# Leonhard111/M3L

Measured on NVIDIA B200. Metric: VTMAE train samples/sec (fwd+bwd+AdamW), higher is better.
Workload: dtype bf16

## Files before the change

### include/m3l_b200.h

```cpp
#ifndef M3L_B200_H_
#define M3L_B200_H_

#include <stddef.h>
#include <stdint.h>

#ifdef __cplusplus
extern "C" {
#endif

const char* m3l_last_error(void);

typedef struct m3l_gemm_args {
  const void* a;
  const void* b;
  int32_t lda, ldb;
  int32_t a_mn_major;
  int32_t b_mn_major;
  int32_t m, n, k;
  int32_t splits;
  int32_t bn;
  void* out;
  int32_t ldo;
  int32_t out_mode;
  const float* bias;
// ... 24 lines not shown
int m3l_gemm_bf16(const m3l_gemm_args* args, void* stream);


typedef struct m3l_ln_mlp_args {
  const void* x;
  int32_t rows, dim, hidden;
  const float* gamma;
  const float* beta;
  float eps;
  const void* w1;
  const float* b1;
  const void* w2;
  const float* b2;
  void* out;
  int32_t out_has_x;
  float* stats;
  void* xn_out;
  void* h_out;
  void* gp_out;
} m3l_ln_mlp_args;

int m3l_ln_mlp_fwd(const m3l_ln_mlp_args* args, void* stream);

#define M3L_MAX_SEGMENTS 8
typedef struct m3l_mask_segments {
  int32_t count;
  int32_t offset[M3L_MAX_SEGMENTS];
  int32_t length[M3L_MAX_SEGMENTS];
  int32_t n_masked[M3L_MAX_SEGMENTS];
} m3l_mask_segments;

int m3l_mask_indices(const float* noise, int batch, int n_total, const m3l_mask_segments* segs,
                     int64_t* masked, int64_t* unmasked, int32_t* slot_of_token,
                     int32_t* unmasked_i32, int32_t* masked_row_of_token, int n_masked_first,
                     void* stream);

typedef struct m3l_patch_source {
  const void* src[4];
  int32_t channels, height, width, patch_h, patch_w;
  int32_t token_base;
  int32_t layout;
  int32_t dtype;
  int64_t stride_b;
  int32_t chan_group;
  int32_t stride_f, stride_ch, stride_y, stride_x;
  float norm_lo, norm_span;
// ... 117 lines not shown
```

### m3l_b200/_lib.py

```python
from __future__ import annotations

import ctypes as C
import os
from pathlib import Path

_LIB_PATH = Path(os.environ.get("M3L_B200_LIB") or (Path(__file__).resolve().parent / "lib" / "libm3l_b200.so"))
_lib = None


class M3LError(RuntimeError):
    pass


class GemmArgs(C.Structure):
    _fields_ = [
        ("a", C.c_void_p), ("b", C.c_void_p),
        ("lda", C.c_int32), ("ldb", C.c_int32),
        ("a_mn_major", C.c_int32), ("b_mn_major", C.c_int32),
        ("m", C.c_int32), ("n", C.c_int32), ("k", C.c_int32),
        ("splits", C.c_int32), ("bn", C.c_int32),
        ("out", C.c_void_p), ("ldo", C.c_int32), ("out_mode", C.c_int32),
        ("bias", C.c_void_p), ("residual", C.c_void_p), ("ldr", C.c_int32),
        ("act", C.c_int32), ("aux_out", C.c_void_p), ("aux_in", C.c_void_p),
        ("ld_aux", C.c_int32), ("alpha", C.c_float), ("colsum_out", C.c_void_p),
        ("out2", C.c_void_p), ("dot_side", C.c_void_p), ("ld_dot", C.c_int32), ("dot_out", C.c_void_p),
        ("ln_x", C.c_void_p), ("ln_stats", C.c_void_p), ("ln_gamma", C.c_void_p), ("ln_skip", C.c_void_p),
        ("ln_dgamma", C.c_void_p), ("ln_dbeta", C.c_void_p), ("ln_dxcol", C.c_void_p),
        ("drop_key", C.c_void_p), ("drop_site", C.c_int32), ("drop_p", C.c_float),
    ]


class LnMlpArgs(C.Structure):
    _fields_ = [
        ("x", C.c_void_p), ("rows", C.c_int32), ("dim", C.c_int32), ("hidden", C.c_int32),
        ("gamma", C.c_void_p), ("beta", C.c_void_p), ("eps", C.c_float),
        ("w1", C.c_void_p), ("b1", C.c_void_p), ("w2", C.c_void_p), ("b2", C.c_void_p),
        ("out", C.c_void_p), ("out_has_x", C.c_int32), ("stats", C.c_void_p), ("xn_out", C.c_void_p),
        ("h_out", C.c_void_p), ("gp_out", C.c_void_p),
    ]


def lib_path() -> Path:
    return _LIB_PATH


def load() -> C.CDLL:
    global _lib
    if _lib is not None:
        return _lib
    if not _LIB_PATH.exists():
        if os.environ.get("M3L_B200_AUTOBUILD", "0") == "1":
            from . import build as _build

            _build.build(verbose=False)
        else:
            raise M3LError(
                f"{_LIB_PATH} not found: the CUDA extension is not built. Run "
                "`python -m m3l_b200.build` (or __graft_entry__.build()); there is no CPU fallback."
            )
    lib = C.CDLL(str(_LIB_PATH))
    lib.m3l_last_error.restype = C.c_char_p
# ... 20 lines not shown
    return C.c_void_p(torch.cuda.current_stream().cuda_stream)


class MaskSegments(C.Structure):
    _fields_ = [("count", C.c_int32), ("offset", C.c_int32 * 8), ("length", C.c_int32 * 8),
                ("n_masked", C.c_int32 * 8)]


class PatchSource(C.Structure):
    _fields_ = [("src", C.c_void_p * 4), ("channels", C.c_int32), ("height", C.c_int32),
                ("width", C.c_int32), ("patch_h", C.c_int32), ("patch_w", C.c_int32),
                ("token_base", C.c_int32),
                ("layout", C.c_int32), ("dtype", C.c_int32), ("stride_b", C.c_int64), ("chan_group", C.c_int32),
                ("stride_f", C.c_int32), ("stride_ch", C.c_int32), ("stride_y", C.c_int32), ("stride_x", C.c_int32),
                ("norm_lo", C.c_float), ("norm_span", C.c_float)]


class MatrixDesc(C.Structure):
    _fields_ = [("src_offset", C.c_int64), ("dst_offset", C.c_int64), ("rows", C.c_int32),
                ("cols", C.c_int32)]


EXPORTED_SYMBOLS = (
    "m3l_last_error", "m3l_gemm_bf16", "m3l_ln_mlp_fwd", "m3l_mask_indices", "m3l_patch_layernorm", "m3l_layernorm_fwd",
    "m3l_layernorm_bwd", "m3l_decoder_assemble_fwd", "m3l_decoder_assemble_bwd", "m3l_rowclass_sum",
    "m3l_mse_loss", "m3l_colsum", "m3l_ln_param_grad", "m3l_attention_fwd", "m3l_attention_bwd",
    "m3l_attention_long_fwd", "m3l_attention_long_bwd",
    "m3l_attention_dh_fwd", "m3l_attention_dh_bwd", "m3l_attention_dropout_fwd", "m3l_attention_dropout_bwd",
    "m3l_dropout_bwd", "m3l_grad_sumsq", "m3l_optimizer_step_begin", "m3l_clip_adamw", "m3l_cast_bf16",
    "m3l_transpose_cast_bf16", "m3l_layerscale_fold", "m3l_layerscale_unfold", "m3l_token_mean_fwd", "m3l_token_mean_bwd",
    "m3l_im2col", "m3l_col2im_relu", "m3l_token_finish", "m3l_token_finish_bwd", "m3l_vt_load", "m3l_patchify", "m3l_row_scatter_add", "m3l_ema_update",
)
```

### m3l_b200/csrc/rowblock.cu

```cuda
#include <stdlib.h>

#include "common.cuh"
#include "m3l_internal.h"

namespace m3l {

namespace {

constexpr int kBM = 128, kD = 256, kCH = 128;
constexpr int kRowWarps = 4, kGeluWarps = 16;
constexpr int kWarps = 2 + kRowWarps + kGeluWarps;
constexpr int kThreads = 32 * kWarps;
constexpr int kKbBytes = 16384;
constexpr int kSlotBytes = 32768;
constexpr int kABytes = 4 * kKbBytes;
constexpr int kStgUnit = 32 * 64;
constexpr int kMaxHidden = 1024;
constexpr int kMaxSlots = 4;

template <bool SAVE>
struct Cfg {
  static constexpr int kSlots = SAVE ? 3 : 4;
  static constexpr int kGeluStg = SAVE ? kGeluWarps * 2048 : 0;
  static constexpr int kSmem = 1024 + kABytes + kSlots * kSlotBytes + kRowWarps * 2 * kStgUnit + kGeluStg +
                               kMaxHidden * 4 + 3 * kD * 4 + 512;
};

struct alignas(8) Bars {
  uint64_t full[kMaxSlots], empty[kMaxSlots];
  uint64_t a_loaded, a_ready, a_free, a_stored;
  uint64_t acc1_full[2], h_full[2], h_read[2];
  uint64_t acc2_full, acc2_empty;
  uint64_t side_full[kRowWarps][2];
  uint32_t tmem_base;
};
static_assert(sizeof(Bars) <= 512, "barrier block");

#ifdef M3L_RB_PROFILE
__device__ long long g_rb_prof[4 * 512];
#define RB_EV(role, idx) do { if (blockIdx.x == 0 && (idx) < 512) g_rb_prof[(role) * 512 + (idx)] = clock64(); } while (0)
#else
#define RB_EV(role, idx) do { } while (0)
#endif

struct Args {
  int M, hidden;
  const float* gamma;
  const float* beta;
  float eps;
  const float* b1;
  const float* b2;
  float* stats;
  int want_xn;
  int out_has_x;
  bf16* out;
};
// ... 69 lines not shown
  }
}
M3L_DEVINL uint4 rb_lds128(uint32_t addr) {
  uint4 v;
  asm volatile("ld.shared.v4.b32 {%0, %1, %2, %3}, [%4];" : "=r"(v.x), "=r"(v.y), "=r"(v.z), "=r"(v.w) : "r"(addr) : "memory");
  return v;
}
M3L_DEVINL float4 rb_lds_f4(uint32_t addr) {
  float4 v;
  asm volatile("ld.shared.v4.f32 {%0, %1, %2, %3}, [%4];" : "=f"(v.x), "=f"(v.y), "=f"(v.z), "=f"(v.w) : "r"(addr));
  return v;
}
M3L_DEVINL void rb_sts128(uint32_t addr, uint4 v) {
  asm volatile("st.shared.v4.b32 [%0], {%1, %2, %3, %4};" ::"r"(addr), "r"(v.x), "r"(v.y), "r"(v.z), "r"(v.w) : "memory");
}

M3L_DEVINL void tile_item(int s, int nc, bool* is_g2, int* c) {
  if (s == 2 * nc - 1) { *is_g2 = true; *c = nc - 1; }
  else if (s < 2) { *is_g2 = false; *c = s; }
  else if ((s & 1) == 0) { *is_g2 = true; *c = (s >> 1) - 1; }
  else { *is_g2 = false; *c = (s + 1) >> 1; }
}

template <bool SAVE>
__global__ void __launch_bounds__(kThreads, 1)
ln_mlp_fwd_kernel(const __grid_constant__ CUtensorMap map_x, const __grid_constant__ CUtensorMap map_w1,
                  const __grid_constant__ CUtensorMap map_w2, const __grid_constant__ CUtensorMap map_x32,
                  const __grid_constant__ CUtensorMap map_out, const __grid_constant__ CUtensorMap map_xn,
                  const __grid_constant__ CUtensorMap map_h, const __grid_constant__ CUtensorMap map_gp, const Args p) {
  using C = Cfg<SAVE>;
  extern __shared__ uint8_t smem_raw[];
  uint8_t* smem = reinterpret_cast<uint8_t*>((reinterpret_cast<uintptr_t>(smem_raw) + 1023) & ~static_cast<uintptr_t>(1023));
  uint8_t* a_tile = smem;
  uint8_t* ring = a_tile + kABytes;
  uint8_t* row_stg = ring + C::kSlots * kSlotBytes;
  uint8_t* gelu_stg = row_stg + kRowWarps * 2 * kStgUnit;
  float* s_b1 = reinterpret_cast<float*>(gelu_stg + C::kGeluStg);
  float* s_gamma = s_b1 + kMaxHidden;
  float* s_beta = s_gamma + kD;
  float* s_b2 = s_beta + kD;
  Bars* bars = reinterpret_cast<Bars*>(s_b2 + kD);
  const uint32_t s_b1_u32 = smem_u32(s_b1), s_gamma_u32 = smem_u32(s_gamma), s_beta_u32 = smem_u32(s_beta),
                 s_b2_u32 = smem_u32(s_b2);

  const int warp = threadIdx.x >> 5, lane = threadIdx.x & 31;
  const int tiles_m = (p.M + kBM - 1) / kBM;
// ... 24 lines not shown
    mbar_init(&bars->acc2_empty, kRowWarps);
    for (int w = 0; w < kRowWarps; ++w) {
      mbar_init(&bars->side_full[w][0], 1);
      mbar_init(&bars->side_full[w][1], 1);
    }
    fence_barrier_init();
  }
  if (warp == 1) tmem_alloc(&bars->tmem_base, 512);
  tc_fence_before_sync();
  __syncthreads();
  tc_fence_after_sync();
  const uint32_t tmem_base = bars->tmem_base;
  pdl_wait();
  for (int i = threadIdx.x; i < p.hidden; i += kThreads) s_b1[i] = p.b1[i];
  if (threadIdx.x < kD) {
    s_gamma[threadIdx.x] = p.gamma[threadIdx.x];
    s_beta[threadIdx.x] = p.beta[threadIdx.x];
    s_b2[threadIdx.x] = p.b2[threadIdx.x];
  }
  __syncthreads();
  pdl_trigger();

  if (warp == 0) {
    if (elect_one()) {
      int slot = 0;
      uint32_t phase = 0;
#pragma unroll 1
      for (int i = 0; i < n_tiles; ++i) {
        const int m0 = ((int)blockIdx.x + i * (int)gridDim.x) * kBM;
        if (i > 0) {
          mbar_wait(&bars->a_free, (i - 1) & 1);
          if (p.want_xn) mbar_wait(&bars->a_stored, (i - 1) & 1);
        }
        mbar_arrive_expect_tx(&bars->a_loaded, kABytes);
#pragma unroll
        for (int kb = 0; kb < 4; ++kb) tma_load_2d(a_tile + kb * kKbBytes, &map_x, &bars->a_loaded, kb * 64, m0);
#pragma unroll 1
        for (int it = 0; it < 2 * nc; ++it) {
          bool is_g2;
          int c;
          tile_item(it, nc, &is_g2, &c);
          const int pc = (c + rot) % nc;
#pragma unroll 1
          for (int q = 0; q < 2; ++q) {
            mbar_wait(&bars->empty[slot], phase ^ 1);
            mbar_arrive_expect_tx(&bars->full[slot], kSlotBytes);
            uint8_t* dst = ring + slot * kSlotBytes;
            if (is_g2) {
              tma_load_2d(dst, &map_w2, &bars->full[slot], pc * kCH + q * 64, 0);
            } else {
              tma_load_2d(dst, &map_w1, &bars->full[slot], (2 * q) * 64, pc * kCH);
              tma_load_2d(dst + kKbBytes, &map_w1, &bars->full[slot], (2 * q + 1) * 64, pc * kCH);
            }
            if (++slot == C::kSlots) { slot = 0; phase ^= 1; }
          }
          RB_EV(0, i * 2 * nc + it);
        }
      }
    }
  } else if (warp == 1) {
    if (elect_one()) {
      constexpr uint32_t idesc1 = umma_idesc_bf16(kBM, 128, 0, 0);
      constexpr uint32_t idesc2 = umma_idesc_bf16(kBM, 256, 0, 0);
      int slot = 0;
      uint32_t phase = 0;
      int gc = 0;
      const uint64_t a_desc0 = umma_smem_desc(smem_u32(a_tile), 16, 1024);
      const uint64_t r_desc0 = umma_smem_desc(smem_u32(ring), 16, 1024);
      const uint32_t d_hi = (uint32_t)(a_desc0 >> 32), a_lo0 = (uint32_t)a_desc0, r_lo0 = (uint32_t)r_desc0;
      auto mk = [&](uint32_t lo) {
        uint64_t d;
        asm("mov.b64 %0, {%1, %2};" : "=l"(d) : "r"(lo), "r"(d_hi));
        return d;
      };
#pragma unroll 1
      for (int i = 0; i < n_tiles; ++i) {
        mbar_wait(&bars->a_ready, i & 1);
        tc_fence_after_sync();
#pragma unroll 1
        for (int it = 0; it < 2 * nc; ++it) {
          bool is_g2;
          int c;
          tile_item(it, nc, &is_g2, &c);
          const int k = gc + c, buf = k & 1;
          if (!is_g2) {
            if (SAVE && k >= 2) {
              mbar_wait(&bars->h_read[buf], ((k - 2) >> 1) & 1);
              tc_fence_after_sync();
            }
            const uint32_t d = tmem_base + buf * 128;
            RB_EV(1, (i * 2 * nc + it) * 2);
#pragma unroll
            for (int q = 0; q < 2; ++q) {
              mbar_wait(&bars->full[slot], phase);
              tc_fence_after_sync();
              const uint32_t b_lo = r_lo0 + slot * (kSlotBytes >> 4);
#pragma unroll
              for (int j = 0; j < 8; ++j) {
                const uint32_t a_off = ((2 * q + (j >> 2)) * kKbBytes + (j & 3) * 32) >> 4;
                const uint32_t b_off = ((j >> 2) * kKbBytes + (j & 3) * 32) >> 4;
                umma_bf16(d, mk(a_lo0 + a_off), mk(b_lo + b_off), idesc1, (q > 0 || j > 0) ? 1u : 0u);
              }
              umma_commit(&bars->empty[slot]);
              if (++slot == C::kSlots) { slot = 0; phase ^= 1; }
            }
            umma_commit(&bars->acc1_full[buf]);
            if (c == nc - 1) umma_commit(&bars->a_free);
            RB_EV(1, (i * 2 * nc + it) * 2 + 1);
          } else {
            mbar_wait(&bars->h_full[buf], (k >> 1) & 1);
            if (c == 0 && i > 0) mbar_wait(&bars->acc2_empty, (i - 1) & 1);
            tc_fence_after_sync();
            RB_EV(1, (i * 2 * nc + it) * 2);
            const uint32_t d = tmem_base + 256;
            const uint32_t h_col = tmem_base + buf * 128;
#pragma unroll
            for (int q = 0; q < 2; ++q) {
              mbar_wait(&bars->full[slot], phase);
              tc_fence_after_sync();
              const uint32_t b_lo = r_lo0 + slot * (kSlotBytes >> 4);
#pragma unroll
              for (int j = 0; j < 4; ++j) {
                const int t = q * 4 + j;
                umma_bf16_ts(d, h_col + 32 * (t >> 1) + 8 * (t & 1), mk(b_lo + ((j * 32) >> 4)), idesc2,
                             (c > 0 || q > 0 || j > 0) ? 1u : 0u);
              }
              umma_commit(&bars->empty[slot]);
              if (++slot == C::kSlots) { slot = 0; phase ^= 1; }
            }
            if (c == nc - 1) umma_commit(&bars->acc2_full);
            RB_EV(1, (i * 2 * nc + it) * 2 + 1);
          }
        }
        gc += nc;
      }
    }
  } else if (warp < 2 + kRowWarps) {
    const int rw = warp - 2;
    const int quad = warp & 3;
    const uint32_t stg = smem_u32(row_stg + rw * 2 * kStgUnit);
    int g_round = 0;
    auto issue_side = [&](int gi, int m0, int r) {
      const int b = gi & 1;
      mbar_arrive_expect_tx(&bars->side_full[rw][b], kStgUnit);
      tma_load_2d_u32(stg + b * kStgUnit, &map_x32, &bars->side_full[rw][b], r * 32, m0 + quad * 32);
    };
    int gc_r = 0;
#pragma unroll 1
    for (int i = 0; i < n_tiles; ++i) {
      const int m0 = ((int)blockIdx.x + i * (int)gridDim.x) * kBM;
      const int row0 = m0 + quad * 32;
      const uint32_t t_acc = tmem_base + (static_cast<uint32_t>(quad * 32) << 16) + 256;
      if (SAVE) {
#pragma unroll 1
        for (int c = 0; c < nc; ++c) {
          const int k = gc_r + c, buf = k & 1;
          const int pc = (c + rot) % nc;
          mbar_wait(&bars->h_full[buf], (k >> 1) & 1);
          tc_fence_after_sync();
// ... 291 lines not shown
  }
  Args p;
  p.M = a->rows; p.hidden = a->hidden;
  p.gamma = a->gamma; p.beta = a->beta; p.eps = a->eps;
  p.b1 = a->b1; p.b2 = a->b2;
  p.stats = a->stats;
  p.want_xn = a->xn_out != nullptr ? 1 : 0;
  p.out = (bf16*)a->out;
  p.out_has_x = (a->out == a->x || a->out_has_x) ? 1 : 0;
  auto kern = ln_mlp_fwd_kernel<SAVE>;
  static bool configured = false;
  if (!configured) {
    M3L_CUDA(cudaFuncSetAttribute(kern, cudaFuncAttributeMaxDynamicSharedMemorySize, C::kSmem));
    configured = true;
  }
  const int tiles = (a->rows + kBM - 1) / kBM;
  const int grid = tiles < device_sm_count() ? tiles : device_sm_count();
  M3L_CUDA(launch_kernel(kern, dim3(grid), dim3(kThreads), C::kSmem, stream, map_x, map_w1, map_w2, map_x32, map_out,
                         map_xn, map_h, map_gp, p));
  M3L_CUDA(cudaGetLastError());
  return M3L_OK;
}

}

}

#ifdef M3L_RB_PROFILE
extern "C" int m3l_debug_rb_prof(long long* host_out, int n) {
  if (n > 4 * 512) return m3l::M3L_ERR_INVALID;
  cudaDeviceSynchronize();
  cudaMemcpyFromSymbol(host_out, m3l::g_rb_prof, n * sizeof(long long));
  static long long zeros[4 * 512];
  cudaMemcpyToSymbol(m3l::g_rb_prof, zeros, sizeof(zeros));
  return m3l::M3L_OK;
}
#endif

extern "C" int m3l_ln_mlp_fwd(const m3l_ln_mlp_args* a, void* stream) {
  using namespace m3l;
  if (a == nullptr) return M3L_ERR_INVALID;
  M3L_REQUIRE(a->dim == kD, "ln_mlp_fwd: dim=%d unsupported (the fused block is built for dim 256)", a->dim);
  M3L_REQUIRE(a->rows > 0 && a->hidden >= kCH && a->hidden <= kMaxHidden && a->hidden % kCH == 0,
              "ln_mlp_fwd: bad shape rows=%d hidden=%d (hidden must be a multiple of 128 up to 1024)", a->rows, a->hidden);
  M3L_REQUIRE(a->x && a->gamma && a->beta && a->w1 && a->b1 && a->w2 && a->b2 && a->out, "ln_mlp_fwd: null pointer");
  M3L_REQUIRE((a->h_out == nullptr) == (a->gp_out == nullptr), "ln_mlp_fwd: h_out and gp_out go together");
  M3L_REQUIRE(a->h_out == nullptr || a->out == a->x || a->out_has_x,
              "ln_mlp_fwd: the training outputs need the accumulate-into-out mode (out == x or out_has_x)");
  if (a->h_out != nullptr) return launch<true>(a, (cudaStream_t)stream);
  return launch<false>(a, (cudaStream_t)stream);
}
```

### m3l_b200/engine.py

```python
from __future__ import annotations

import contextlib
import gc
from dataclasses import dataclass, field
from typing import Dict, List, Optional, Tuple

import torch

from . import ops
from .arena import ParamArena

import os

_SM_COUNT_CACHE = {}


def _sm_count() -> int:
    dev = torch.cuda.current_device() if torch.cuda.is_available() else -1
    n = _SM_COUNT_CACHE.get(dev)
    if n is None:
        n = _SM_COUNT_CACHE[dev] = torch.cuda.get_device_properties(dev).multi_processor_count if dev >= 0 else 148
    return n
_FUSED_MLP = os.environ.get("M3L_FUSED_MLP", "1") != "0"
_FUSED_LN_BWD = os.environ.get("M3L_FUSED_LN_BWD", "1") != "0"
_FUSED_LN_BWD_MIN_ROWS = int(os.environ.get("M3L_FUSED_LN_BWD_MIN_ROWS", "16384"))


def _dgrad_ln_bwd(dy_in, w_t, x, stats, gamma, dgamma, dbeta, skip, dx_colsum):
    if _FUSED_LN_BWD and x.shape[1] == 256 and x.shape[0] >= _FUSED_LN_BWD_MIN_ROWS:
        return ops.gemm(dy_in, w_t, ln_bwd=dict(x=x, stats=stats, gamma=gamma, skip=skip, dgamma=dgamma, dbeta=dbeta,
                                               dx_colsum=dx_colsum))
    dxn = ops.gemm(dy_in, w_t)
    return ops.layernorm_bwd(dxn, x, stats, gamma, dgamma=dgamma, dbeta=dbeta, skip=skip, dx_colsum=dx_colsum)


@dataclass
class StackSpec:
    prefix: str
    dim: int
    depth: int
    heads: int
    dim_head: int
    mlp_dim: int

    @property
    def inner(self):
        return self.heads * self.dim_head

# ... 148 lines not shown
        x = x_out
    return x


def last_ff_bias(spec: StackSpec) -> str:
    return f"{spec.prefix}.layers.{spec.depth - 1}.1.net.4.bias"


def stack_dx_colsum(G: GradView, spec: StackSpec, saved: list) -> Optional[torch.Tensor]:
    return None if saved[-1][-1] is not None else G(last_ff_bias(spec))


def stack_bwd(A: ParamArena, G: GradView, spec: StackSpec, dx: torch.Tensor, B: int, n: int, saved: list):
    scale = spec.dim_head ** -0.5
    M = dx.shape[0]
    fork = WgradFork(A.device)
    for l in reversed(range(spec.depth)):
        pa, pf = f"{spec.prefix}.layers.{l}.0", f"{spec.prefix}.layers.{l}.1"
        x, xn1, st1, qkv, o, lse, x_mid, xn2, st2, pre, h, drop = saved[l]
        dy = dx
        if drop is not None:
            dy = ops.dropout_bwd(dx, drop(l, 3), colsum=G(pf + ".net.4.bias"))
        fork.wgrad(dy, h, G(pf + ".net.4.weight"))
        dpre = ops.gemm(dy, A.bf_t(pf + ".net.4.weight"), act=ops.GELU_BWD, aux_in=pre,
                        colsum_out=G(pf + ".net.1.bias"))
        fork.wgrad(dpre, xn2, G(pf + ".net.1.weight"))
        dx_mid = _dgrad_ln_bwd(dpre, A.bf_t(pf + ".net.1.weight"), x_mid, st2, A.f32(pf + ".net.0.weight"),
                               G(pf + ".net.0.weight"), G(pf + ".net.0.bias"), dx,
                               G(pa + ".to_out.0.bias") if drop is None else None)
        dy_mid = dx_mid
        if drop is not None:
            dy_mid = ops.dropout_bwd(dx_mid, drop(l, 1), colsum=G(pa + ".to_out.0.bias"))
        fork.wgrad(dy_mid, o, G(pa + ".to_out.0.weight"))
        delta = torch.empty((M, spec.heads), dtype=torch.float32, device=dx.device) if spec.dim_head == 64 else None
        do = ops.gemm(dy_mid, A.bf_t(pa + ".to_out.0.weight"), dot_side=o if delta is not None else None, dot_out=delta)
        dqkv = ops.mha_bwd(qkv, o, do, lse, B, n, spec.heads, spec.dim_head, scale, delta=delta,
                           dropout=drop(l, 0) if drop else None)
        fork.wgrad(dqkv, xn1, G(pa + ".to_qkv.weight"))
        prev_bias = G(f"{spec.prefix}.layers.{l - 1}.1.net.4.bias") if (l > 0 and drop is None) else None
        dx_in = _dgrad_ln_bwd(dqkv, A.bf_t(pa + ".to_qkv.weight"), x, st1, A.f32(pa + ".norm.weight"),
                              G(pa + ".norm.weight"), G(pa + ".norm.bias"), dx_mid, prev_bias)
        fork.join()
        dx = dx_in
    return dx


@dataclass
class Geometry:
    use_vision: bool
    nt: int
    n_img: int
    n_tac: int
# ... 444 lines not shown
```

### m3l_b200/ops.py

```python
from __future__ import annotations

import ctypes as C
from typing import NamedTuple, Optional

import torch

from . import _lib
from ._lib import GemmArgs, check, current_stream, ptr

GELU_FWD = 1
GELU_BWD = 2
RELU = 3


class Dropout(NamedTuple):
    key: torch.Tensor
    site: int
    p: float


def _drop_args(d: Optional[Dropout]):
    if d is None:
        return C.c_void_p(0), 0, C.c_float(0.0)
    assert d.key.dtype == torch.int64 and d.key.is_cuda and d.key.numel() >= 1
# ... 98 lines not shown
        if save:
            out, out_has_x = x.clone(), True
        else:
            out = torch.empty_like(x)
    assert out.shape == x.shape and out.dtype == torch.bfloat16 and out.is_contiguous()
    a = _lib.LnMlpArgs()
    a.x, a.rows, a.dim, a.hidden = ptr(x), M, D, hidden
    a.gamma, a.beta, a.eps = ptr(gamma), ptr(beta), eps
    a.w1, a.b1, a.w2, a.b2 = ptr(w1), ptr(b1), ptr(w2), ptr(b2)
    a.out, a.out_has_x = ptr(out), int(out_has_x)
    stats = xn = h = gp = None
    if save:
        stats = torch.empty((M, 2), dtype=torch.float32, device=x.device)
        xn = torch.empty_like(x)
        h = torch.empty((M, hidden), dtype=torch.bfloat16, device=x.device)
        gp = torch.empty_like(h)
        a.stats, a.xn_out, a.h_out, a.gp_out = ptr(stats), ptr(xn), ptr(h), ptr(gp)
    check(_lib.load().m3l_ln_mlp_fwd(C.byref(a), current_stream()), "m3l_ln_mlp_fwd")
    if save:
        return out, stats, xn, h, gp
    return out


def make_segments(segs):
    s = _lib.MaskSegments()
    s.count = len(segs)
    for i, (o, l, m) in enumerate(segs):
        s.offset[i], s.length[i], s.n_masked[i] = o, l, m
    return s


def mask_indices(noise: torch.Tensor, segs, want_slots: bool = True, extra: bool = False, n_masked_first: int = 0):
    _req_cuda(noise)
    assert noise.dtype == torch.float32 and noise.is_contiguous()
    B, n = noise.shape
    nm = sum(m for _, _, m in segs)
    nu = sum(l - m for _, l, m in segs)
    masked = torch.empty((B, nm), dtype=torch.int64, device=noise.device)
    unmasked = torch.empty((B, nu), dtype=torch.int64, device=noise.device)
    slots = torch.empty((B, n), dtype=torch.int32, device=noise.device) if want_slots else None
    cs = make_segments(segs)
    u32 = torch.empty((B, nu), dtype=torch.int32, device=noise.device) if extra else None
    mrow = torch.empty((B, n), dtype=torch.int32, device=noise.device) if extra else None
    check(_lib.load().m3l_mask_indices(ptr(noise), B, n, C.byref(cs), ptr(masked), ptr(unmasked), ptr(slots),
                                       ptr(u32), ptr(mrow), n_masked_first, current_stream()), "m3l_mask_indices")
    if extra:
# ... 444 lines not shown
```

Baseline: 110,400.

## Fuse MLP backward GEMMs with GELU grad and LayerNorm backward in one kernel

Adds a persistent tcgen05 kernel that computes dy·W2ᵀ, applies the GELU gradient, writes dpre, then multiplies by W1ᵀ in TMEM and finishes the LayerNorm backward in the same pass. It accumulates db1, dgamma, dbeta and the residual colsum with atomics. The aim is to drop the separate dgrad GEMM and LN-backward launches and the HBM round trip of dpre as a GEMM input. The producer and MMA-issuer loops are factored into shared device helpers so forward and backward reuse them. Atomics on parameter grads and the more complex synchronisation add risk.

```diff
diff --git a/include/m3l_b200.h b/include/m3l_b200.h
--- a/include/m3l_b200.h
+++ b/include/m3l_b200.h
@@ -70,6 +70,25 @@
 
 int m3l_ln_mlp_fwd(const m3l_ln_mlp_args* args, void* stream);
 
+typedef struct m3l_ln_mlp_bwd_args {
+  const void* dy;
+  int32_t rows, dim, hidden;
+  const void* x;
+  const float* stats;
+  const float* gamma;
+  const void* w1_t;
+  const void* w2_t;
+  const void* gelu_grad;
+  void* dpre;
+  void* dx;
+  float* db1;
+  float* dgamma;
+  float* dbeta;
+  float* dx_colsum;
+} m3l_ln_mlp_bwd_args;
+
+int m3l_ln_mlp_bwd(const m3l_ln_mlp_bwd_args* args, void* stream);
+
 #define M3L_MAX_SEGMENTS 8
 typedef struct m3l_mask_segments {
   int32_t count;
diff --git a/m3l_b200/_lib.py b/m3l_b200/_lib.py
--- a/m3l_b200/_lib.py
+++ b/m3l_b200/_lib.py
@@ -37,6 +37,15 @@
         ("w1", C.c_void_p), ("b1", C.c_void_p), ("w2", C.c_void_p), ("b2", C.c_void_p),
         ("out", C.c_void_p), ("out_has_x", C.c_int32), ("stats", C.c_void_p), ("xn_out", C.c_void_p),
         ("h_out", C.c_void_p), ("gp_out", C.c_void_p),
+    ]
+
+
+class LnMlpBwdArgs(C.Structure):
+    _fields_ = [
+        ("dy", C.c_void_p), ("rows", C.c_int32), ("dim", C.c_int32), ("hidden", C.c_int32),
+        ("x", C.c_void_p), ("stats", C.c_void_p), ("gamma", C.c_void_p), ("w1_t", C.c_void_p), ("w2_t", C.c_void_p),
+        ("gelu_grad", C.c_void_p), ("dpre", C.c_void_p), ("dx", C.c_void_p), ("db1", C.c_void_p),
+        ("dgamma", C.c_void_p), ("dbeta", C.c_void_p), ("dx_colsum", C.c_void_p),
     ]
 
 
@@ -103,7 +112,7 @@
 
 
 EXPORTED_SYMBOLS = (
-    "m3l_last_error", "m3l_gemm_bf16", "m3l_ln_mlp_fwd", "m3l_mask_indices", "m3l_patch_layernorm", "m3l_layernorm_fwd",
+    "m3l_last_error", "m3l_gemm_bf16", "m3l_ln_mlp_fwd", "m3l_ln_mlp_bwd", "m3l_mask_indices", "m3l_patch_layernorm", "m3l_layernorm_fwd",
     "m3l_layernorm_bwd", "m3l_decoder_assemble_fwd", "m3l_decoder_assemble_bwd", "m3l_rowclass_sum",
     "m3l_mse_loss", "m3l_colsum", "m3l_ln_param_grad", "m3l_attention_fwd", "m3l_attention_bwd",
     "m3l_attention_long_fwd", "m3l_attention_long_bwd",
diff --git a/m3l_b200/csrc/rowblock.cu b/m3l_b200/csrc/rowblock.cu
--- a/m3l_b200/csrc/rowblock.cu
+++ b/m3l_b200/csrc/rowblock.cu
@@ -32,6 +32,7 @@
   uint64_t acc1_full[2], h_full[2], h_read[2];
   uint64_t acc2_full, acc2_empty;
   uint64_t side_full[kRowWarps][2];
+  uint64_t unit_full[kGeluWarps][2];
   uint32_t tmem_base;
 };
 static_assert(sizeof(Bars) <= 512, "barrier block");
@@ -147,6 +148,124 @@
   else { *is_g2 = false; *c = (s + 1) >> 1; }
 }
 
+template <int kSlots>
+M3L_DEVINL void rb_produce(const CUtensorMap* map_a, const CUtensorMap* map_g1, const CUtensorMap* map_g2, Bars* bars,
+                           uint8_t* a_tile, uint8_t* ring, int n_tiles, int nc, int rot, uint64_t* a_stored) {
+  int slot = 0;
+  uint32_t phase = 0;
+#pragma unroll 1
+  for (int i = 0; i < n_tiles; ++i) {
+    const int m0 = ((int)blockIdx.x + i * (int)gridDim.x) * kBM;
+    if (i > 0) {
+      mbar_wait(&bars->a_free, (i - 1) & 1);
+      if (a_stored != nullptr) mbar_wait(a_stored, (i - 1) & 1);
+    }
+    mbar_arrive_expect_tx(&bars->a_loaded, kABytes);
+#pragma unroll
+    for (int kb = 0; kb < 4; ++kb) tma_load_2d(a_tile + kb * kKbBytes, map_a, &bars->a_loaded, kb * 64, m0);
+#pragma unroll 1
+    for (int it = 0; it < 2 * nc; ++it) {
+      bool is_g2;
+      int c;
+      tile_item(it, nc, &is_g2, &c);
+      const int pc = (c + rot) % nc;
+#pragma unroll 1
+      for (int q = 0; q < 2; ++q) {
+        mbar_wait(&bars->empty[slot], phase ^ 1);
+        mbar_arrive_expect_tx(&bars->full[slot], kSlotBytes);
+        uint8_t* dst = ring + slot * kSlotBytes;
+        if (is_g2) {
+          tma_load_2d(dst, map_g2, &bars->full[slot], pc * kCH + q * 64, 0);
+        } else {
+          tma_load_2d(dst, map_g1, &bars->full[slot], (2 * q) * 64, pc * kCH);
+          tma_load_2d(dst + kKbBytes, map_g1, &bars->full[slot], (2 * q + 1) * 64, pc * kCH);
+        }
+        if (++slot == kSlots) { slot = 0; phase ^= 1; }
+      }
+      RB_EV(0, i * 2 * nc + it);
+    }
+  }
+}
+
+template <int kSlots, bool WAIT_H_READ>
+M3L_DEVINL void rb_issue_products(Bars* bars, uint64_t* a_ready, uint8_t* a_tile, uint8_t* ring, uint32_t tmem_base,
+                                  int n_tiles, int nc) {
+  constexpr uint32_t idesc1 = umma_idesc_bf16(kBM, 128, 0, 0);
+  constexpr uint32_t idesc2 = umma_idesc_bf16(kBM, 256, 0, 0);
+  int slot = 0;
+  uint32_t phase = 0;
+  int gc = 0;
+  const uint64_t a_desc0 = umma_smem_desc(smem_u32(a_tile), 16, 1024);
+  const uint64_t r_desc0 = umma_smem_desc(smem_u32(ring), 16, 1024);
+  const uint32_t d_hi = (uint32_t)(a_desc0 >> 32), a_lo0 = (uint32_t)a_desc0, r_lo0 = (uint32_t)r_desc0;
+  auto mk = [&](uint32_t lo) {
+    uint64_t d;
+    asm("mov.b64 %0, {%1, %2};" : "=l"(d) : "r"(lo), "r"(d_hi));
+    return d;
+  };
+#pragma unroll 1
+  for (int i = 0; i < n_tiles; ++i) {
+    mbar_wait(a_ready, i & 1);
+    tc_fence_after_sync();
+#pragma unroll 1
+    for (int it = 0; it < 2 * nc; ++it) {
+      bool is_g2;
+      int c;
+      tile_item(it, nc, &is_g2, &c);
+      const int k = gc + c, buf = k & 1;
+      if (!is_g2) {
+        if (WAIT_H_READ && k >= 2) {
+          mbar_wait(&bars->h_read[buf], ((k - 2) >> 1) & 1);
+          tc_fence_after_sync();
+        }
+        const uint32_t d = tmem_base + buf * 128;
+        RB_EV(1, (i * 2 * nc + it) * 2);
+#pragma unroll
+        for (int q = 0; q < 2; ++q) {
+          mbar_wait(&bars->full[slot], phase);
+          tc_fence_after_sync();
+          const uint32_t b_lo = r_lo0 + slot * (kSlotBytes >> 4);
+#pragma unroll
+          for (int j = 0; j < 8; ++j) {
+            const uint32_t a_off = ((2 * q + (j >> 2)) * kKbBytes + (j & 3) * 32) >> 4;
+            const uint32_t b_off = ((j >> 2) * kKbBytes + (j & 3) * 32) >> 4;
+            umma_bf16(d, mk(a_lo0 + a_off), mk(b_lo + b_off), idesc1, (q > 0 || j > 0) ? 1u : 0u);
+          }
+          umma_commit(&bars->empty[slot]);
+          if (++slot == kSlots) { slot = 0; phase ^= 1; }
+        }
+        umma_commit(&bars->acc1_full[buf]);
+        if (c == nc - 1) umma_commit(&bars->a_free);
+        RB_EV(1, (i * 2 * nc + it) * 2 + 1);
+      } else {
+        mbar_wait(&bars->h_full[buf], (k >> 1) & 1);
+        if (c == 0 && i > 0) mbar_wait(&bars->acc2_empty, (i - 1) & 1);
+        tc_fence_after_sync();
+        RB_EV(1, (i * 2 * nc + it) * 2);
+        const uint32_t d = tmem_base + 256;
+        const uint32_t h_col = tmem_base + buf * 128;
+#pragma unroll
+        for (int q = 0; q < 2; ++q) {
+          mbar_wait(&bars->full[slot], phase);
+          tc_fence_after_sync();
+          const uint32_t b_lo = r_lo0 + slot * (kSlotBytes >> 4);
+#pragma unroll
+          for (int j = 0; j < 4; ++j) {
+            const int t = q * 4 + j;
+            umma_bf16_ts(d, h_col + 32 * (t >> 1) + 8 * (t & 1), mk(b_lo + ((j * 32) >> 4)), idesc2,
+                         (c > 0 || q > 0 || j > 0) ? 1u : 0u);
+          }
+          umma_commit(&bars->empty[slot]);
+          if (++slot == kSlots) { slot = 0; phase ^= 1; }
+        }
+        if (c == nc - 1) umma_commit(&bars->acc2_full);
+        RB_EV(1, (i * 2 * nc + it) * 2 + 1);
+      }
+    }
+    gc += nc;
+  }
+}
+
 template <bool SAVE>
 __global__ void __launch_bounds__(kThreads, 1)
 ln_mlp_fwd_kernel(const __grid_constant__ CUtensorMap map_x, const __grid_constant__ CUtensorMap map_w1,
@@ -217,119 +336,11 @@
   pdl_trigger();
 
   if (warp == 0) {
-    if (elect_one()) {
-      int slot = 0;
-      uint32_t phase = 0;
-#pragma unroll 1
-      for (int i = 0; i < n_tiles; ++i) {
-        const int m0 = ((int)blockIdx.x + i * (int)gridDim.x) * kBM;
-        if (i > 0) {
-          mbar_wait(&bars->a_free, (i - 1) & 1);
-          if (p.want_xn) mbar_wait(&bars->a_stored, (i - 1) & 1);
-        }
-        mbar_arrive_expect_tx(&bars->a_loaded, kABytes);
-#pragma unroll
-        for (int kb = 0; kb < 4; ++kb) tma_load_2d(a_tile + kb * kKbBytes, &map_x, &bars->a_loaded, kb * 64, m0);
-#pragma unroll 1
-        for (int it = 0; it < 2 * nc; ++it) {
-          bool is_g2;
-          int c;
-          tile_item(it, nc, &is_g2, &c);
-          const int pc = (c + rot) % nc;
-#pragma unroll 1
-          for (int q = 0; q < 2; ++q) {
-            mbar_wait(&bars->empty[slot], phase ^ 1);
-            mbar_arrive_expect_tx(&bars->full[slot], kSlotBytes);
-            uint8_t* dst = ring + slot * kSlotBytes;
-            if (is_g2) {
-              tma_load_2d(dst, &map_w2, &bars->full[slot], pc * kCH + q * 64, 0);
-            } else {
-              tma_load_2d(dst, &map_w1, &bars->full[slot], (2 * q) * 64, pc * kCH);
-              tma_load_2d(dst + kKbBytes, &map_w1, &bars->full[slot], (2 * q + 1) * 64, pc * kCH);
-            }
-            if (++slot == C::kSlots) { slot = 0; phase ^= 1; }
-          }
-          RB_EV(0, i * 2 * nc + it);
-        }
-      }
-    }
+    if (elect_one())
+      rb_produce<C::kSlots>(&map_x, &map_w1, &map_w2, bars, a_tile, ring, n_tiles, nc, rot,
+                            p.want_xn ? &bars->a_stored : nullptr);
   } else if (warp == 1) {
-    if (elect_one()) {
-      constexpr uint32_t idesc1 = umma_idesc_bf16(kBM, 128, 0, 0);
-      constexpr uint32_t idesc2 = umma_idesc_bf16(kBM, 256, 0, 0);
-      int slot = 0;
-      uint32_t phase = 0;
-      int gc = 0;
-      const uint64_t a_desc0 = umma_smem_desc(smem_u32(a_tile), 16, 1024);
-      const uint64_t r_desc0 = umma_smem_desc(smem_u32(ring), 16, 1024);
-      const uint32_t d_hi = (uint32_t)(a_desc0 >> 32), a_lo0 = (uint32_t)a_desc0, r_lo0 = (uint32_t)r_desc0;
-      auto mk = [&](uint32_t lo) {
-        uint64_t d;
-        asm("mov.b64 %0, {%1, %2};" : "=l"(d) : "r"(lo), "r"(d_hi));
-        return d;
-      };
-#pragma unroll 1
-      for (int i = 0; i < n_tiles; ++i) {
-        mbar_wait(&bars->a_ready, i & 1);
-        tc_fence_after_sync();
-#pragma unroll 1
-        for (int it = 0; it < 2 * nc; ++it) {
-          bool is_g2;
-          int c;
-          tile_item(it, nc, &is_g2, &c);
-          const int k = gc + c, buf = k & 1;
-          if (!is_g2) {
-            if (SAVE && k >= 2) {
-              mbar_wait(&bars->h_read[buf], ((k - 2) >> 1) & 1);
-              tc_fence_after_sync();
-            }
-            const uint32_t d = tmem_base + buf * 128;
-            RB_EV(1, (i * 2 * nc + it) * 2);
-#pragma unroll
-            for (int q = 0; q < 2; ++q) {
-              mbar_wait(&bars->full[slot], phase);
-              tc_fence_after_sync();
-              const uint32_t b_lo = r_lo0 + slot * (kSlotBytes >> 4);
-#pragma unroll
-              for (int j = 0; j < 8; ++j) {
-                const uint32_t a_off = ((2 * q + (j >> 2)) * kKbBytes + (j & 3) * 32) >> 4;
-                const uint32_t b_off = ((j >> 2) * kKbBytes + (j & 3) * 32) >> 4;
-                umma_bf16(d, mk(a_lo0 + a_off), mk(b_lo + b_off), idesc1, (q > 0 || j > 0) ? 1u : 0u);
-              }
-              umma_commit(&bars->empty[slot]);
-              if (++slot == C::kSlots) { slot = 0; phase ^= 1; }
-            }
-            umma_commit(&bars->acc1_full[buf]);
-            if (c == nc - 1) umma_commit(&bars->a_free);
-            RB_EV(1, (i * 2 * nc + it) * 2 + 1);
-          } else {
-            mbar_wait(&bars->h_full[buf], (k >> 1) & 1);
-            if (c == 0 && i > 0) mbar_wait(&bars->acc2_empty, (i - 1) & 1);
-            tc_fence_after_sync();
-            RB_EV(1, (i * 2 * nc + it) * 2);
-            const uint32_t d = tmem_base + 256;
-            const uint32_t h_col = tmem_base + buf * 128;
-#pragma unroll
-            for (int q = 0; q < 2; ++q) {
-              mbar_wait(&bars->full[slot], phase);
-              tc_fence_after_sync();
-              const uint32_t b_lo = r_lo0 + slot * (kSlotBytes >> 4);
-#pragma unroll
-              for (int j = 0; j < 4; ++j) {
-                const int t = q * 4 + j;
-                umma_bf16_ts(d, h_col + 32 * (t >> 1) + 8 * (t & 1), mk(b_lo + ((j * 32) >> 4)), idesc2,
-                             (c > 0 || q > 0 || j > 0) ? 1u : 0u);
-              }
-              umma_commit(&bars->empty[slot]);
-              if (++slot == C::kSlots) { slot = 0; phase ^= 1; }
-            }
-            if (c == nc - 1) umma_commit(&bars->acc2_full);
-            RB_EV(1, (i * 2 * nc + it) * 2 + 1);
-          }
-        }
-        gc += nc;
-      }
-    }
+    if (elect_one()) rb_issue_products<C::kSlots, SAVE>(bars, &bars->a_ready, a_tile, ring, tmem_base, n_tiles, nc);
   } else if (warp < 2 + kRowWarps) {
     const int rw = warp - 2;
     const int quad = warp & 3;
@@ -667,6 +678,352 @@
   return M3L_OK;
 }
 
+constexpr int kBwdWarps = 2 + kGeluWarps;
+constexpr int kBwdThreads = 32 * kBwdWarps;
+struct BwdCfg {
+  static constexpr int kSlots = 3;
+  static constexpr int kSmem = 1024 + kABytes + kSlots * kSlotBytes + kGeluWarps * 2 * kStgUnit + 512;
+};
+
+struct BwdArgs {
+  int M, hidden;
+  const float* stats;
+  const float* gamma;
+  float* db1;
+  float* dgamma;
+  float* dbeta;
+  float* dxcol;
+};
+
+M3L_DEVINL float rb_colsum16(float (&v)[16], int lane) {
+#pragma unroll
+  for (int off = 8; off >= 1; off >>= 1) {
+    const bool hi = (lane & off) != 0;
+#pragma unroll
+    for (int i = 0; i < off; ++i) {
+      const float send = hi ? v[i] : v[i + off];
+      const float keep = hi ? v[i + off] : v[i];
+      v[i] = keep + __shfl_xor_sync(0xffffffffu, send, off);
+    }
+  }
+  return v[0] + __shfl_xor_sync(0xffffffffu, v[0], 16);
+}
+M3L_DEVINL float rb_colsum32(float (&v)[32], int lane) {
+#pragma unroll
+  for (int off = 16; off >= 1; off >>= 1) {
+    const bool hi = (lane & off) != 0;
+#pragma unroll
+    for (int i = 0; i < off; ++i) {
+      const float send = hi ? v[i] : v[i + off];
+      const float keep = hi ? v[i + off] : v[i];
+      v[i] = keep + __shfl_xor_sync(0xffffffffu, send, off);
+    }
+  }
+  return v[0];
+}
+
+__global__ void __launch_bounds__(kBwdThreads, 1)
+ln_mlp_bwd_kernel(const __grid_constant__ CUtensorMap map_dy, const __grid_constant__ CUtensorMap map_w2t,
+                  const __grid_constant__ CUtensorMap map_w1t, const __grid_constant__ CUtensorMap map_gp,
+                  const __grid_constant__ CUtensorMap map_dpre, const __grid_constant__ CUtensorMap map_x32,
+                  const __grid_constant__ CUtensorMap map_dy32, const __grid_constant__ CUtensorMap map_dx,
+                  const BwdArgs p) {
+  extern __shared__ uint8_t smem_raw[];
+  uint8_t* smem = reinterpret_cast<uint8_t*>((reinterpret_cast<uintptr_t>(smem_raw) + 1023) & ~static_cast<uintptr_t>(1023));
+  uint8_t* a_tile = smem;
+  uint8_t* ring = a_tile + kABytes;
+  uint8_t* units = ring + BwdCfg::kSlots * kSlotBytes;
+  Bars* bars = reinterpret_cast<Bars*>(units + kGeluWarps * 2 * kStgUnit);
+
+  const int warp = threadIdx.x >> 5, lane = threadIdx.x & 31;
+  const int tiles_m = (p.M + kBM - 1) / kBM;
+  const int n_tiles = (int)blockIdx.x < tiles_m ? (tiles_m - (int)blockIdx.x + (int)gridDim.x - 1) / (int)gridDim.x : 0;
+  const int nc = p.hidden / kCH;
+  const int rot = (int)blockIdx.x % nc;
+
+  if (warp == 0 && lane == 0) {
+    tma_prefetch_desc(&map_dy);
+    tma_prefetch_desc(&map_w2t);
+    tma_prefetch_desc(&map_w1t);
+    tma_prefetch_desc(&map_gp);
+    tma_prefetch_desc(&map_dpre);
+    for (int s = 0; s < BwdCfg::kSlots; ++s) {
+      mbar_init(&bars->full[s], 1);
+      mbar_init(&bars->empty[s], 1);
+    }
+    mbar_init(&bars->a_loaded, 1);
+    mbar_init(&bars->a_free, 1);
+    for (int b = 0; b < 2; ++b) {
+      mbar_init(&bars->acc1_full[b], 1);
+      mbar_init(&bars->h_full[b], kGeluWarps);
+    }
+    mbar_init(&bars->acc2_full, 1);
+    mbar_init(&bars->acc2_empty, kGeluWarps);
+    for (int w = 0; w < kGeluWarps; ++w) {
+      mbar_init(&bars->unit_full[w][0], 1);
+      mbar_init(&bars->unit_full[w][1], 1);
+    }
+    fence_barrier_init();
+  }
+  if (warp == 1) tmem_alloc(&bars->tmem_base, 512);
+  tc_fence_before_sync();
+  __syncthreads();
+  tc_fence_after_sync();
+  const uint32_t tmem_base = bars->tmem_base;
+  pdl_wait();
+  pdl_trigger();
+
+  if (warp == 0) {
+    if (elect_one()) rb_produce<BwdCfg::kSlots>(&map_dy, &map_w2t, &map_w1t, bars, a_tile, ring, n_tiles, nc, rot, nullptr);
+  } else if (warp == 1) {
+    if (elect_one()) rb_issue_products<BwdCfg::kSlots, false>(bars, &bars->a_loaded, a_tile, ring, tmem_base, n_tiles, nc);
+  } else {
+    const int gw = warp - 2;
+    const int quad = warp & 3;
+    const int part = gw >> 2;
+    const uint32_t unit0 = smem_u32(units + gw * 2 * kStgUnit);
+    const int sw = (lane >> 1) & 3;
+    uint32_t uses0 = 0, uses1 = 0;
+    auto unit = [&](int b) { return unit0 + b * kStgUnit; };
+    auto unit_wait = [&](int b) {
+      if (b == 0) { mbar_wait(&bars->unit_full[gw][0], uses0 & 1); ++uses0; }
+      else { mbar_wait(&bars->unit_full[gw][1], uses1 & 1); ++uses1; }
+    };
+    auto load_item = [&](int s, int k0, int row0) {
+      const int b = (k0 + s) & 1;
+      tma_wait_group_read<0>();
+      fence_proxy_async_smem();
+      mbar_arrive_expect_tx(&bars->unit_full[gw][b], kStgUnit);
+      if (s < nc) tma_load_2d_u32(unit(b), &map_gp, &bars->unit_full[gw][b], ((s + rot) % nc) * kCH + part * 32, row0);
+      else tma_load_2d_u32(unit(b), &map_x32, &bars->unit_full[gw][b], part * 64 + b * 32, row0);
+    };
+    int gc = 0;
+    if (n_tiles > 0 && elect_one()) {
+      const int row0 = (int)blockIdx.x * kBM + quad * 32;
+      load_item(0, 0, row0);
+      load_item(1, 0, row0);
+    }
+    __syncwarp();
+#pragma unroll 1
+    for (int i = 0; i < n_tiles; ++i) {
+      const int m0 = ((int)blockIdx.x + i * (int)gridDim.x) * kBM;
+      const int row0 = m0 + quad * 32;
+#pragma unroll 1
+      for (int c = 0; c < nc; ++c) {
+        const int k = gc + c, buf = k & 1, b = k & 1;
+        const int pc = (c + rot) % nc;
+        mbar_wait(&bars->acc1_full[buf], (k >> 1) & 1);
+        tc_fence_after_sync();
+        if (gw == 0 && lane == 0) RB_EV(3, k * 4);
+        const uint32_t taddr = tmem_base + (static_cast<uint32_t>(quad * 32) << 16) + buf * 128 + part * 32;
+        uint32_t v[32];
+        tmem_ld_32x32(taddr, v);
+        unit_wait(b);
+        uint32_t g[16];
+#pragma unroll
+        for (int j = 0; j < 4; ++j) {
+          const uint4 u = rb_lds128(unit(b) + lane * 64 + ((j ^ sw) << 4));
+          g[4 * j] = u.x; g[4 * j + 1] = u.y; g[4 * j + 2] = u.z; g[4 * j + 3] = u.w;
+        }
+        tmem_ld_wait();
+        if (gw == 0 && lane == 0) RB_EV(3, k * 4 + 1);
+        uint32_t w[16];
+#pragma unroll
+        for (int j = 0; j < 16; ++j) {
+          float d0, d1;
+          f2_unpack(f2_mul(f2_packu(v[2 * j], v[2 * j + 1]), f2_packu(g[j] << 16, g[j] & 0xffff0000u)), d0, d1);
+          w[j] = pack_bf16x2(d0, d1);
+        }
+        tmem_st_32x16(taddr, w);
+#pragma unroll
+        for (int j = 0; j < 4; ++j)
+          rb_sts128(unit(b) + lane * 64 + ((j ^ sw) << 4), make_uint4(w[4 * j], w[4 * j + 1], w[4 * j + 2], w[4 * j + 3]));
+        fence_proxy_async_smem();
+        tmem_st_wait();
+        tc_fence_before_sync();
+        __syncwarp();
+        if (lane == 0) mbar_arrive(&bars->h_full[buf]);
+        if (gw == 0 && lane == 0) RB_EV(3, k * 4 + 2);
+        if (elect_one()) {
+          tma_store_2d(&map_dpre, unit(b), pc * kCH + part * 32, row0);
+          tma_commit_group();
+        }
+        float cs[32];
+#pragma unroll
+        for (int j = 0; j < 16; ++j) {
+          const float2 d = unpack_bf16x2(w[j]);
+          cs[2 * j] = d.x; cs[2 * j + 1] = d.y;
+        }
+        atomicAdd(p.db1 + pc * kCH + part * 32 + lane, rb_colsum32(cs, lane));
+        if (elect_one()) load_item(c + 2, gc, row0);
+        __syncwarp();
+        if (gw == 0 && lane == 0) RB_EV(3, k * 4 + 3);
+      }
+      const int my_row = row0 + lane;
+      const bool in = my_row < p.M;
+      float mean = 0.f, rstd = 0.f;
+      if (in) {
+        const float2 ms = __ldg(reinterpret_cast<const float2*>(p.stats) + my_row);
+        mean = ms.x; rstd = ms.y;
+      }
+      const float* gam = p.gamma + part * 64;
+      mbar_wait(&bars->acc2_full, i & 1);
+      tc_fence_after_sync();
+      if (gw == 0 && lane == 0) RB_EV(2, i * 4 + 2);
+      const uint32_t t_acc = tmem_base + (static_cast<uint32_t>(quad * 32) << 16) + 256 + part * 64;
+      uint32_t xw[32];
+      float s1 = 0.f, s2 = 0.f;
+#pragma unroll
+      for (int gi = 0; gi < 2; ++gi) {
+        uint32_t v[32];
+        tmem_ld_32x32(t_acc + gi * 32, v);
+        unit_wait(gi);
+#pragma unroll
+        for (int j = 0; j < 4; ++j) {
+          const uint4 u = rb_lds128(unit(gi) + lane * 64 + ((j ^ sw) << 4));
+          xw[gi * 16 + 4 * j] = u.x; xw[gi * 16 + 4 * j + 1] = u.y; xw[gi * 16 + 4 * j + 2] = u.z; xw[gi * 16 + 4 * j + 3] = u.w;
+        }
+        tmem_ld_wait();
+#pragma unroll
+        for (int j = 0; j < 32; j += 4) {
+          const float4 gm = __ldg(reinterpret_cast<const float4*>(gam + gi * 32 + j));
+          const float2 x01 = unpack_bf16x2(xw[gi * 16 + (j >> 1)]), x23 = unpack_bf16x2(xw[gi * 16 + (j >> 1) + 1]);
+          const float g0 = __uint_as_float(v[j]) * gm.x, g1 = __uint_as_float(v[j + 1]) * gm.y;
+          const float g2 = __uint_as_float(v[j + 2]) * gm.z, g3 = __uint_as_float(v[j + 3]) * gm.w;
+          s1 += (g0 + g1) + (g2 + g3);
+          s2 = fmaf(g0, (x01.x - mean) * rstd, s2);
+          s2 = fmaf(g1, (x01.y - mean) * rstd, s2);
+          s2 = fmaf(g2, (x23.x - mean) * rstd, s2);
+          s2 = fmaf(g3, (x23.y - mean) * rstd, s2);
+        }
+      }
+      __syncwarp();
+      asm volatile("st.shared.v2.f32 [%0], {%1, %2};" ::"r"(unit(0) + lane * 8), "f"(s1), "f"(s2) : "memory");
+      named_bar_sync(1 + quad, 4 * 32);
+      float S1 = 0.f, S2 = 0.f;
+#pragma unroll
+      for (int q = 0; q < 4; ++q) {
+        float a, bb;
+        asm volatile("ld.shared.v2.f32 {%0, %1}, [%2];" : "=f"(a), "=f"(bb)
+                     : "r"(smem_u32(units + (q * 4 + (gw & 3)) * 2 * kStgUnit) + lane * 8) : "memory");
+        S1 += a; S2 += bb;
+      }
+      named_bar_sync(1 + quad, 4 * 32);
+      const float c1 = S1 * (1.0f / kD), c2 = S2 * (1.0f / kD);
+      if (elect_one()) {
+        fence_proxy_async_smem();
+#pragma unroll
+        for (int gi = 0; gi < 2; ++gi) {
+          mbar_arrive_expect_tx(&bars->unit_full[gw][gi], kStgUnit);
+          tma_load_2d_u32(unit(gi), &map_dy32, &bars->unit_full[gw][gi], part * 64 + gi * 32, row0);
+        }
+      }
+      __syncwarp();
+#pragma unroll
+      for (int gi = 0; gi < 2; ++gi) {
+        unit_wait(gi);
+#pragma unroll
+        for (int h = 0; h < 2; ++h) {
+          uint32_t v[16];
+          tmem_ld_32x16(t_acc + gi * 32 + h * 16, v);
+          tmem_ld_wait();
+          if (gi == 1 && h == 1) {
+            tc_fence_before_sync();
+            __syncwarp();
+            if (lane == 0) mbar_arrive(&bars->acc2_empty);
+          }
+          const uint32_t a0 = unit(gi) + lane * 64 + (((2 * h) ^ sw) << 4), a1 = unit(gi) + lane * 64 + (((2 * h + 1) ^ sw) << 4);
+          const uint4 k0 = rb_lds128(a0), k1 = rb_lds128(a1);
+          const uint32_t sk[8] = {k0.x, k0.y, k0.z, k0.w, k1.x, k1.y, k1.z, k1.w};
+          float a_c[16];
+          uint32_t o[8];
+#pragma unroll
+          for (int j = 0; j < 16; j += 2) {
+            const float2 gm = __ldg(reinterpret_cast<const float2*>(gam + gi * 32 + h * 16 + j));
+            const float2 xv = unpack_bf16x2(xw[gi * 16 + h * 8 + (j >> 1)]), kv = unpack_bf16x2(sk[j >> 1]);
+            const float dy0 = in ? __uint_as_float(v[j]) : 0.f, dy1 = in ? __uint_as_float(v[j + 1]) : 0.f;
+            const float xh0 = (xv.x - mean) * rstd, xh1 = (xv.y - mean) * rstd;
+            const float dx0 = in ? fmaf(rstd, dy0 * gm.x - c1 - xh0 * c2, kv.x) : 0.f;
+            const float dx1 = in ? fmaf(rstd, dy1 * gm.y - c1 - xh1 * c2, kv.y) : 0.f;
+            a_c[j] = dx0; a_c[j + 1] = dx1;
+            v[j] = __float_as_uint(dy0); v[j + 1] = __float_as_uint(dy1);
+            o[j >> 1] = pack_bf16x2(dx0, dx1);
+          }
+          rb_sts128(a0, make_uint4(o[0], o[1], o[2], o[3]));
+          rb_sts128(a1, make_uint4(o[4], o[5], o[6], o[7]));
+          const float tc = rb_colsum16(a_c, lane);
+          float a_g[16], a_b[16];
+#pragma unroll
+          for (int j = 0; j < 16; j += 2) {
+            const float2 xv = unpack_bf16x2(xw[gi * 16 + h * 8 + (j >> 1)]);
+            a_g[j] = __uint_as_float(v[j]) * ((xv.x - mean) * rstd);
+            a_g[j + 1] = __uint_as_float(v[j + 1]) * ((xv.y - mean) * rstd);
+            a_b[j] = __uint_as_float(v[j]); a_b[j + 1] = __uint_as_float(v[j + 1]);
+          }
+          const float tg = rb_colsum16(a_g, lane), tb = rb_colsum16(a_b, lane);
+          if (lane < 16) {
+            const int col = part * 64 + gi * 32 + h * 16 + lane;
+            atomicAdd(p.dgamma + col, tg);
+            atomicAdd(p.dbeta + col, tb);
+            if (p.dxcol != nullptr) atomicAdd(p.dxcol + col, tc);
+          }
+        }
+        fence_proxy_async_smem();
+        __syncwarp();
+        if (elect_one()) {
+          tma_store_2d(&map_dx, unit(gi), part * 64 + gi * 32, row0);
+          tma_commit_group();
+        }
+      }
+      if (gw == 0 && lane == 0) RB_EV(2, i * 4 + 3);
+      gc += nc;
+      if (i + 1 < n_tiles && elect_one()) {
+        const int row0n = m0 + (int)gridDim.x * kBM + quad * 32;
+        load_item(0, gc, row0n);
+        load_item(1, gc, row0n);
+      }
+      __syncwarp();
+    }
+    tma_wait_group_read<0>();
+  }
+
+  tc_fence_before_sync();
+  __syncthreads();
+  if (warp == 1) {
+    tc_fence_after_sync();
+    tmem_dealloc(tmem_base, 512);
+  }
+}
+
+int launch_bwd(const m3l_ln_mlp_bwd_args* a, cudaStream_t stream) {
+  static_assert(BwdCfg::kSmem <= 227 * 1024, "shared memory budget");
+  CUtensorMap map_dy, map_w2t, map_w1t, map_gp, map_dpre, map_x32, map_dy32, map_dx;
+  int s;
+  if ((s = make_tmap_2d_bf16(&map_dy, a->dy, a->rows, kD, kD, 128))) return s;
+  if ((s = make_tmap_2d_bf16(&map_w2t, a->w2_t, a->hidden, kD, kD, 128))) return s;
+  if ((s = make_tmap_2d_bf16(&map_w1t, a->w1_t, kD, a->hidden, a->hidden, 256))) return s;
+  if ((s = make_tmap_2d_bf16_sw64(&map_gp, a->gelu_grad, a->rows, a->hidden, a->hidden, 32))) return s;
+  if ((s = make_tmap_2d_bf16_sw64(&map_dpre, a->dpre, a->rows, a->hidden, a->hidden, 32))) return s;
+  if ((s = make_tmap_2d_bf16_sw64(&map_x32, a->x, a->rows, kD, kD, 32))) return s;
+  if ((s = make_tmap_2d_bf16_sw64(&map_dy32, a->dy, a->rows, kD, kD, 32))) return s;
+  if ((s = make_tmap_2d_bf16_sw64(&map_dx, a->dx, a->rows, kD, kD, 32))) return s;
+  BwdArgs p;
+  p.M = a->rows; p.hidden = a->hidden;
+  p.stats = a->stats; p.gamma = a->gamma;
+  p.db1 = a->db1; p.dgamma = a->dgamma; p.dbeta = a->dbeta; p.dxcol = a->dx_colsum;
+  static bool configured = false;
+  if (!configured) {
+    M3L_CUDA(cudaFuncSetAttribute(ln_mlp_bwd_kernel, cudaFuncAttributeMaxDynamicSharedMemorySize, BwdCfg::kSmem));
+    configured = true;
+  }
+  const int tiles = (a->rows + kBM - 1) / kBM;
+  const int grid = tiles < device_sm_count() ? tiles : device_sm_count();
+  M3L_CUDA(launch_kernel(ln_mlp_bwd_kernel, dim3(grid), dim3(kBwdThreads), BwdCfg::kSmem, stream, map_dy, map_w2t, map_w1t,
+                         map_gp, map_dpre, map_x32, map_dy32, map_dx, p));
+  M3L_CUDA(cudaGetLastError());
+  return M3L_OK;
+}
+
 }
 
 }
@@ -695,3 +1052,15 @@
   if (a->h_out != nullptr) return launch<true>(a, (cudaStream_t)stream);
   return launch<false>(a, (cudaStream_t)stream);
 }
+
+extern "C" int m3l_ln_mlp_bwd(const m3l_ln_mlp_bwd_args* a, void* stream) {
+  using namespace m3l;
+  if (a == nullptr) return M3L_ERR_INVALID;
+  M3L_REQUIRE(a->dim == kD, "ln_mlp_bwd: dim=%d unsupported (the fused block is built for dim 256)", a->dim);
+  M3L_REQUIRE(a->rows > 0 && a->hidden >= kCH && a->hidden <= kMaxHidden && a->hidden % kCH == 0,
+              "ln_mlp_bwd: bad shape rows=%d hidden=%d (hidden must be a multiple of 128 up to 1024)", a->rows, a->hidden);
+  M3L_REQUIRE(a->dy && a->x && a->stats && a->gamma && a->w1_t && a->w2_t && a->gelu_grad && a->dpre && a->dx && a->db1 &&
+                  a->dgamma && a->dbeta,
+              "ln_mlp_bwd: null pointer");
+  return launch_bwd(a, (cudaStream_t)stream);
+}
diff --git a/m3l_b200/engine.py b/m3l_b200/engine.py
--- a/m3l_b200/engine.py
+++ b/m3l_b200/engine.py
@@ -24,6 +24,7 @@
 _FUSED_MLP = os.environ.get("M3L_FUSED_MLP", "1") != "0"
 _FUSED_LN_BWD = os.environ.get("M3L_FUSED_LN_BWD", "1") != "0"
 _FUSED_LN_BWD_MIN_ROWS = int(os.environ.get("M3L_FUSED_LN_BWD_MIN_ROWS", "16384"))
+_FUSED_MLP_BWD = os.environ.get("M3L_FUSED_MLP_BWD", "1") != "0"
 
 
 def _dgrad_ln_bwd(dy_in, w_t, x, stats, gamma, dgamma, dbeta, skip, dx_colsum):
@@ -218,12 +219,20 @@
         if drop is not None:
             dy = ops.dropout_bwd(dx, drop(l, 3), colsum=G(pf + ".net.4.bias"))
         fork.wgrad(dy, h, G(pf + ".net.4.weight"))
-        dpre = ops.gemm(dy, A.bf_t(pf + ".net.4.weight"), act=ops.GELU_BWD, aux_in=pre,
-                        colsum_out=G(pf + ".net.1.bias"))
-        fork.wgrad(dpre, xn2, G(pf + ".net.1.weight"))
-        dx_mid = _dgrad_ln_bwd(dpre, A.bf_t(pf + ".net.1.weight"), x_mid, st2, A.f32(pf + ".net.0.weight"),
-                               G(pf + ".net.0.weight"), G(pf + ".net.0.bias"), dx,
-                               G(pa + ".to_out.0.bias") if drop is None else None)
+        if (_FUSED_MLP_BWD and _FUSED_LN_BWD and drop is None and ops.ln_mlp_supported(spec.dim, spec.mlp_dim)
+                and M >= _FUSED_LN_BWD_MIN_ROWS):
+            dx_mid, dpre = ops.ln_mlp_bwd(dy, x_mid, st2, A.f32(pf + ".net.0.weight"), A.bf_t(pf + ".net.1.weight"),
+                                          A.bf_t(pf + ".net.4.weight"), pre, db1=G(pf + ".net.1.bias"),
+                                          dgamma=G(pf + ".net.0.weight"), dbeta=G(pf + ".net.0.bias"),
+                                          dx_colsum=G(pa + ".to_out.0.bias"))
+            fork.wgrad(dpre, xn2, G(pf + ".net.1.weight"))
+        else:
+            dpre = ops.gemm(dy, A.bf_t(pf + ".net.4.weight"), act=ops.GELU_BWD, aux_in=pre,
+                            colsum_out=G(pf + ".net.1.bias"))
+            fork.wgrad(dpre, xn2, G(pf + ".net.1.weight"))
+            dx_mid = _dgrad_ln_bwd(dpre, A.bf_t(pf + ".net.1.weight"), x_mid, st2, A.f32(pf + ".net.0.weight"),
+                                   G(pf + ".net.0.weight"), G(pf + ".net.0.bias"), dx,
+                                   G(pa + ".to_out.0.bias") if drop is None else None)
         dy_mid = dx_mid
         if drop is not None:
             dy_mid = ops.dropout_bwd(dx_mid, drop(l, 1), colsum=G(pa + ".to_out.0.bias"))
diff --git a/m3l_b200/ops.py b/m3l_b200/ops.py
--- a/m3l_b200/ops.py
+++ b/m3l_b200/ops.py
@@ -144,6 +144,27 @@
     return out
 
 
+def ln_mlp_bwd(dy, x, stats, gamma, w1_t, w2_t, gelu_grad, *, db1, dgamma, dbeta, dx_colsum=None):
+    _req_cuda(dy, x, stats, gamma, w1_t, w2_t, gelu_grad, db1, dgamma, dbeta, dx_colsum)
+    M, D = dy.shape
+    hidden = w2_t.shape[0]
+    for t in (dy, x, w1_t, w2_t, gelu_grad):
+        assert t.dtype == torch.bfloat16 and t.is_contiguous()
+    assert x.shape == (M, D) and w1_t.shape == (D, hidden) and w2_t.shape == (hidden, D) and gelu_grad.shape == (M, hidden)
+    assert stats.shape == (M, 2) and stats.dtype == torch.float32 and stats.is_contiguous()
+    for t, n in ((gamma, D), (dgamma, D), (dbeta, D), (dx_colsum, D), (db1, hidden)):
+        assert t is None or (t.dtype == torch.float32 and t.is_contiguous() and t.numel() == n)
+    dx = torch.empty_like(dy)
+    dpre = torch.empty_like(gelu_grad)
+    a = _lib.LnMlpBwdArgs()
+    a.dy, a.rows, a.dim, a.hidden = ptr(dy), M, D, hidden
+    a.x, a.stats, a.gamma, a.w1_t, a.w2_t, a.gelu_grad = ptr(x), ptr(stats), ptr(gamma), ptr(w1_t), ptr(w2_t), ptr(gelu_grad)
+    a.dpre, a.dx = ptr(dpre), ptr(dx)
+    a.db1, a.dgamma, a.dbeta, a.dx_colsum = ptr(db1), ptr(dgamma), ptr(dbeta), ptr(dx_colsum)
+    check(_lib.load().m3l_ln_mlp_bwd(C.byref(a), current_stream()), "m3l_ln_mlp_bwd")
+    return dx, dpre
+
+
 def make_segments(segs):
     s = _lib.MaskSegments()
     s.count = len(segs)
```

Measured after the change: 112,100, median of 6. 1.01x the previous value.
